# lvclark/tagdigger

Measured on AMD Instinct MI355X. Metric: FASTQ reads/sec (whole node), 200M-read × 100k-tag synthetic, 1/2/4/8 MI355X, higher is better.
Workload: dtype u8; 1 GPU; BASELINE configs[2] shape, device-resident (tier T1): 200000000 reads x 384 barcodes x 100000 tags per GPU, 100 bp reads, 219 B/record, cut site TGCAG, one library per GPU; reads_per_gpu=200000000, barcodes=384, tags=100000, fastq_bytes_per_gpu=43800000000

## Files before the change

tagdigger_amd/csrc/inst_fast4.hip:

```cpp
#include <hip/hip_runtime.h>
#define TD_INST_ONLY 1
#include "kernel_fast4.hpp"
#define X(W, NQ) template __global__ void tdk::k_fast4<W, NQ, (TD_INST_PROG != 0)>(const tdk::FParams);
TD_FAST2_COMBOS(X)
#undef X
```

tagdigger_amd/csrc/kernel_fast4.hpp:

```cpp
#pragma once
#include "kernel_fast2.hpp"

namespace tdk {

#ifndef TD_F4_WAVES
#define TD_F4_WAVES 16
#endif
#ifndef TD_F4_NPROD
#define TD_F4_NPROD 11
#endif
#ifndef TD_F4_SLOTS
#define TD_F4_SLOTS 5
#endif
constexpr int F4_PROD = 4 , F4_WAVES = TD_F4_WAVES, F4_BLOCK = 64 * F4_WAVES;
#ifndef TD_F4_CPT
#define TD_F4_CPT 6
#endif
constexpr int F4_CPT = TD_F4_CPT;
constexpr uint32_t F4_WCH = F4_CPT * 64;
constexpr uint32_t F4_WBYTES = F4_WCH * 16;
constexpr uint32_t F4_TILE = F4_PROD * F4_WBYTES;
constexpr int F4_SLOTS = TD_F4_SLOTS;
constexpr uint32_t F4_SPIN_LIMIT = 1u << 18;
#ifndef TD_F4_EAGER_MIN
#define TD_F4_EAGER_MIN 65
#endif
#ifndef TD_F4_EAGER_SPINS
#define TD_F4_EAGER_SPINS 4
#endif
#ifndef TD_F4_P_CONS
#define TD_F4_P_CONS 1
#endif

enum { F4_DONE = 0, F4_FREE = 1, F4_REMAIN = 2, F4_FLAGS = 3, F4_TOT = 4 , F4_VOTE = 8 , F4_R0 = 12, F4_WB1 = 13, F4_WB2 = 14,
       F4_WB3 = 15, F4_TOTAL = 16, F4_SEQ = 17, F4_NCUM = 18, F4_NWANT = 19, F4_TIDX = 20, F4_CTRL_DW = 24 };
constexpr uint32_t F4_FLAG_HI = 1, F4_FLAG_OVER = 2, F4_FLAG_HALO_HI = 4;
constexpr uint32_t F4_ABORT_DW = F4_SLOTS * F4_CTRL_DW, F4_READY_DW = F4_ABORT_DW + 1, F4_AVAIL_DW = F4_ABORT_DW + 2, F4_CLAIMED_DW = F4_ABORT_DW + 3;
constexpr uint32_t F4_NPROD_MIN = 7, F4_NPROD_MAX = 13;
constexpr uint32_t F4_CTRL_BYTES = 1024;
static_assert(F4_CLAIMED_DW < 240 && F4_WAVES <= 16, "hand-off words");

__device__ __forceinline__ uint32_t lds_ld(const uint32_t *p) { return __hip_atomic_load(p, __ATOMIC_RELAXED, __HIP_MEMORY_SCOPE_WORKGROUP); }
__device__ __forceinline__ void lds_st(uint32_t *p, uint32_t v) { __hip_atomic_store(p, v, __ATOMIC_RELAXED, __HIP_MEMORY_SCOPE_WORKGROUP); }
__device__ __forceinline__ bool f4_wait(uint32_t *p, uint32_t need, uint32_t *abort_word, unsigned long long *stats) {
    for (uint32_t spins = 0;; spins++) {
        const uint32_t v = lds_ld(p);
        if (v >= need) break;
        if (spins > F4_SPIN_LIMIT || lds_ld(abort_word)) {
            lds_st(abort_word, 1u);
            if ((threadIdx.x & 63) == 0) atomicOr(stats + ST_ERR, ERR_SPIN);
            return false;
        }
        __builtin_amdgcn_s_sleep(1);
    }
    asm volatile("s_waitcnt lgkmcnt(0)" ::: "memory");
    return true;
}

#ifndef TD_INST_ONLY
__global__ __launch_bounds__(256) void k_f4_estimate(const uint8_t *buf, uint64_t nbytes, uint32_t *out) {
    __shared__ uint32_t total;
    if (threadIdx.x == 0) total = 0;
    __syncthreads();
    const uint32_t n = (uint32_t)(nbytes < 65536ull ? nbytes : 65536ull) & ~15u;
    uint32_t cnt = 0;
    for (uint32_t i = threadIdx.x * 16u; i < n; i += 256u * 16u) {
        const uint4 v = *reinterpret_cast<const uint4 *>(buf + i);
        cnt += (uint32_t)__builtin_popcount(eq_mask16(v, 0x0A0A0A0Au) | eq_mask16(v, 0x0D0D0D0Du));
    }
    atomicAdd(&total, cnt);
    __syncthreads();
    if (threadIdx.x == 0) {
        const uint32_t rec = total >= 8u ? 4u * n / total : 219u;
        *out = rec < 150u ? 8u : rec < 195u ? 9u : rec < 270u ? 10u : rec < 420u ? 11u : 12u;
    }
}
#endif

#ifdef TD_PHASE_PROF
#define F4_STAMP(i) do { const unsigned long long now_ = __builtin_amdgcn_s_memtime(); f4acc[i] += now_ - f4last; f4last = now_; } while (0)
#else
#define F4_STAMP(i) do {} while (0)
#endif

template <int W, int NQ, bool PROG>
__global__ __launch_bounds__(F4_BLOCK, F4_WAVES / 4) void k_fast4(const FParams fp) {
    const KParams &p = fp.k;
#ifdef TD_PHASE_PROF
    unsigned long long f4acc[12] = {};
    unsigned long long f4last = __builtin_amdgcn_s_memtime();
#endif
    constexpr uint32_t TILE = F4_TILE, WCH = F4_WCH, WBYTES = F4_WBYTES;
    constexpr int CPT = F4_CPT;
    static_assert(W <= 3, "k_fast4 has the pipelined probe of the 64-byte buckets only");

    extern __shared__ __attribute__((aligned(16))) uint8_t lds[];
    const uint32_t halo = p.halo;
    const uint32_t slot_bytes = TILE + halo;
    uint8_t *L_raw0 = lds;
    uint16_t *L_list0 = reinterpret_cast<uint16_t *>(lds + F4_SLOTS * slot_bytes);
    uint32_t *L_ctrl = reinterpret_cast<uint32_t *>(lds + F4_SLOTS * slot_bytes + F4_SLOTS * F4_PROD * WCH * 2u);
    uint32_t *L_abort = L_ctrl + F4_ABORT_DW;
    uint8_t *L_hc = reinterpret_cast<uint8_t *>(L_ctrl) + F4_CTRL_BYTES;
    uint8_t *L_bidx = L_hc + ((uint32_t)F4_WAVES - F4_NPROD_MIN) * HC_BYTES_PER_WAVE;
    TileCtx cx{nullptr, 0u, reinterpret_cast<const unsigned long long *>(L_bidx),
               reinterpret_cast<const uint32_t *>(L_bidx + p.off_bmeta),
               reinterpret_cast<const uint16_t *>(L_bidx + p.off_bdir)};

    const int tid = threadIdx.x, lane = tid & 63;
    const int wave = __builtin_amdgcn_readfirstlane(tid >> 6);
    for (uint32_t i = tid; i < p.bblob_bytes / 4; i += F4_BLOCK)
        reinterpret_cast<uint32_t *>(L_bidx)[i] = p.bblob[i];
    if (tid < (int)(F4_CTRL_BYTES / 4)) L_ctrl[tid] = 0;
    __syncthreads();

    const unsigned long long carried = p.cursor_in ? *p.cursor_in : 0ull;
    const uint64_t first_line = p.first_line + carried;
    const uint32_t nwork = p.ntiles;
    const uint32_t RUN = p.run ? p.run : 1u;
    auto tile_base = [&](uint32_t tile) -> const uint8_t * {
        return tile >= p.tail_tile ? p.tail_buf + (uint64_t)(tile - p.tail_tile) * TILE : p.buf + (uint64_t)tile * TILE;
    };
    typedef uint32_t u32x4 __attribute__((ext_vector_type(4)));
    auto tile_rsrc = [&](uint32_t tile) {
        return __builtin_amdgcn_make_buffer_rsrc(const_cast<uint8_t *>(tile_base(tile)), 0, (int)(TILE + 4096u), 0x00020000);
    };

    uint32_t np_ = p.f4_nprod ? p.f4_nprod : (p.f4_nprod_dev ? *p.f4_nprod_dev : (uint32_t)TD_F4_NPROD);
    np_ = np_ < F4_NPROD_MIN ? F4_NPROD_MIN : np_ > F4_NPROD_MAX ? F4_NPROD_MAX : np_;
    const uint32_t NPROD = (uint32_t)__builtin_amdgcn_readfirstlane((int)np_);
    {
        uint4 va[CPT], vb[CPT];
        u32x4 vha, vhb;
        auto fetch_job = [&](uint4 (&v)[CPT], u32x4 &vh, uint32_t tile, uint32_t q) {
            const uint32_t voff = q * WBYTES + (uint32_t)lane * 16u;
            const bool hh = q == (uint32_t)F4_PROD - 1u && (uint32_t)lane < halo / 16u;
            const uint32_t hoff = hh ? (uint32_t)lane * 16u : 0x40000000u;
            const __amdgpu_buffer_rsrc_t rs = tile_rsrc(tile);
#pragma unroll
            for (int j = 0; j < CPT; j++) {
                const u32x4 qq = __builtin_amdgcn_raw_buffer_load_b128(rs, voff, j * 1024, 2 );
                v[j] = make_uint4(qq.x, qq.y, qq.z, qq.w);
            }
            vh = __builtin_amdgcn_raw_buffer_load_b128(rs, hoff, (int)TILE, 0);
        };
        auto tile_of = [&](uint32_t k) -> uint32_t { return (k / RUN) * (gridDim.x * RUN) + blockIdx.x * RUN + k % RUN; };
        uint32_t n_local = 0;
        for (uint32_t first = blockIdx.x * RUN; first < nwork; first += gridDim.x * RUN) n_local += min(RUN, nwork - first);
        uint32_t my_job = (uint32_t)wave;
        if (wave < (int)NPROD) {
            if (my_job < 4u * n_local) fetch_job(va, vha, tile_of(my_job >> 2), my_job & 3u);
            if (my_job + NPROD < 4u * n_local) fetch_job(vb, vhb, tile_of((my_job + NPROD) >> 2), (my_job + NPROD) & 3u);
        }
        uint32_t *g_ready = L_ctrl + F4_READY_DW, *g_avail = L_ctrl + F4_AVAIL_DW, *g_claimed = L_ctrl + F4_CLAIMED_DW;

        if (wave < (int)NPROD) {
        auto produce = [&](uint4 (&v)[CPT], u32x4 &vh, const uint32_t k, const uint32_t t) -> bool {
            const uint32_t qtr = my_job & 3u;
            const uint32_t voff = qtr * WBYTES + (uint32_t)lane * 16u;
            const bool has_halo = qtr == (uint32_t)F4_PROD - 1u && (uint32_t)lane < halo / 16u;
            const uint32_t slot = k % (uint32_t)F4_SLOTS, use = k / (uint32_t)F4_SLOTS;
            uint8_t *L_raw = L_raw0 + slot * slot_bytes;
            uint16_t *Ll = L_list0 + (slot * F4_PROD + qtr) * WCH;
            uint32_t *ctrl = L_ctrl + slot * F4_CTRL_DW;
            const uint64_t tbase = (uint64_t)t * TILE;
            const bool carry_ok = k % RUN != 0u && t != 1u;
            const uint32_t job2 = my_job + 2u * NPROD;
            const bool more = job2 < 4u * n_local;
            const uint32_t t2 = more ? tile_of(job2 >> 2) : 0u;
            F4_STAMP(4);
            if (!f4_wait(ctrl + F4_FREE, use, L_abort, p.stats)) return false;
            F4_STAMP(0);
            bool wave_crb = false;
            uint32_t myflags = 0;
            {
                uint32_t hiacc = 0;
#pragma unroll
                for (int j = 0; j < CPT; j++) hiacc |= v[j].x | v[j].y | v[j].z | v[j].w;
#pragma unroll
                for (int j = 0; j < CPT; j++) *reinterpret_cast<uint4 *>(L_raw + voff + j * 1024) = v[j];
                uint16_t *Lm = Ll + lane;
                const bool general = __any((hiacc & 0x80808080u) != 0);
                if (__builtin_expect(!general, 1)) {
                    uint32_t cr_absent = 0x80808080u;
#pragma unroll
                    for (int j = 0; j < CPT; j++) cr_absent_ascii(v[j], cr_absent);
                    const bool has_cr = __any((cr_absent & 0x80808080u) != 0x80808080u);
                    if (__builtin_expect(!has_cr, 1)) {
#pragma unroll
                        for (int j = 0; j < CPT; j++) Lm[j * 64] = (uint16_t)nl_mask16_ascii(v[j]);
                    } else {
                        uint32_t crs = 0;
#pragma unroll
                        for (int j = 0; j < CPT; j++) {
                            const uint32_t nl = eq_mask16_ascii(v[j], 0x0A0A0A0Au, 0x7F7F7F7Fu), cr = eq_mask16_ascii(v[j], 0x0D0D0D0Du, 0x7F7F7F7Fu);
// ... 2 lines not shown
                        }
                        wave_crb = __any((crs & 0x8000u) != 0);
                    }
                } else {
                    uint32_t crs = 0;
#pragma unroll
                    for (int j = 0; j < CPT; j++) {
                        const uint32_t nl = eq_mask16(v[j], 0x0A0A0A0Au), cr = eq_mask16(v[j], 0x0D0D0D0Du);
                        Lm[j * 64] = (uint16_t)(nl | (cr & ~(nl >> 1)));
                        crs |= cr;
                    }
                    wave_crb = __any((crs & 0x8000u) != 0);
                    myflags |= F4_FLAG_HI;
                }
            }
            if (has_halo) *reinterpret_cast<uint4 *>(L_raw + TILE + (uint32_t)lane * 16u) = make_uint4(vh.x, vh.y, vh.z, vh.w);
            if (qtr == (uint32_t)F4_PROD - 1u && __any(has_halo && ((vh.x | vh.y | vh.z | vh.w) & 0x80808080u) != 0)) myflags |= F4_FLAG_HALO_HI;
            const uint32_t my_qtr = qtr;
            if (more) fetch_job(v, vh, t2, job2 & 3u);
            wave_lds_fence();
            F4_STAMP(1);

            uint32_t mm[CPT / 2];
#pragma unroll
            for (int i = 0; i < CPT / 2; i++) mm[i] = reinterpret_cast<const uint32_t *>(Ll)[lane * (CPT / 2) + i];
            const uint32_t span0 = my_qtr * WBYTES + (uint32_t)lane * (CPT * 16u);
            const uint32_t wend = (my_qtr + 1u) * WBYTES;
            if (__builtin_expect(wave_crb, 0)) {
#pragma unroll
                for (int i = 0; i < CPT / 2; i++) {
#pragma unroll
                    for (int hbit = 15; hbit < 32; hbit += 16) {
                        if ((mm[i] >> hbit) & 1u) {
                            const uint32_t at = span0 + 32u * i + (uint32_t)hbit;
                            if (L_raw[at] == 0x0Du) {
                                const uint32_t nx = at + 1u < wend ? (uint32_t)L_raw[at + 1u] : (uint32_t)tile_base(t)[at + 1u];
                                if (nx == 0x0Au) mm[i] &= ~(1u << hbit);
                            }
                        }
                    }
                }
            }
            uint32_t cnt = 0;
#pragma unroll
            for (int i = 0; i < CPT / 2; i++) cnt += __builtin_popcount(mm[i]);
            const uint32_t incl = wave_incl_scan(cnt, lane);
            const uint32_t wtot = (uint32_t)__builtin_amdgcn_readlane((int)incl, 63);
            uint32_t packed = 0;
            if (!carry_ok) {
                uint32_t fpos = 0;
                bool found = false;
// ... 90 lines not shown
                asm volatile("s_waitcnt lgkmcnt(0)" ::: "memory");
                if (lane == 0)
                    __hip_atomic_store(reinterpret_cast<unsigned long long *>(ctrl + F4_NCUM), (unsigned long long)ncum | ((unsigned long long)nwant << 32),
                                       __ATOMIC_RELAXED, __HIP_MEMORY_SCOPE_WORKGROUP);
                asm volatile("s_waitcnt lgkmcnt(0)" ::: "memory");
                if (lane == 0) {
                    lds_st(g_avail, ncum + nwant);
                    if (nwant == 0u) lds_st(ctrl + F4_FREE, use + 1u);
                }
                asm volatile("s_waitcnt lgkmcnt(0)" ::: "memory");
                if (lane == 0) lds_st(g_ready, k + 1u);
                F4_STAMP(3);
            }
            return true;
        };
            for (;;) {
                if (!(my_job < 4u * n_local)) break;
                if (!produce(va, vha, my_job >> 2, tile_of(my_job >> 2))) break;
                my_job += NPROD;
                if (!(my_job < 4u * n_local)) break;
                if (!produce(vb, vhb, my_job >> 2, tile_of(my_job >> 2))) break;
                my_job += NPROD;
            }
        } else {
        const int cons = wave < (int)NPROD ? 0 : wave - (int)NPROD;
        uint2 *hcS = reinterpret_cast<uint2 *>(L_hc + cons * HC_BYTES_PER_WAVE);
        uint8_t *hcE = L_hc + cons * HC_BYTES_PER_WAVE + HC_SLOTS * 8;
        if (wave >= (int)NPROD) {
#pragma unroll
            for (int q = 0; q < HC_SLOTS / 64; q++) hcS[q * 64 + lane] = make_uint2(HC_EMPTY, 0u);
            wave_lds_fence();
        }
        bool hc_on = p.hot_cache != 0;
        uint32_t hc_hits = 0, hc_rest = 0, aged = 0;
        int st_reads = 0, st_bar = 0, st_tag = 0;
        Pending<W> pd;
        Pending<W> nx;
        bool pd_valid = false;
        bool phit_tag = false;
        auto finish_pending = [&](bool &hit, uint32_t &cell) {
            vm_settled();
            const uint64_t res = match_finish<W>(p, pd);
            const uint32_t kind = (uint32_t)(res >> 62);
// ... 146 lines not shown
                    break;
                }
                __builtin_amdgcn_s_sleep(1);
            }
            settle();
            if (p.hot_cache) hc_flush(p.counts, hcS, (uint32_t)lane);
            unsigned long long r = wave_sum64((unsigned long long)(long long)st_reads), b = wave_sum64((unsigned long long)(long long)st_bar),
                               g = wave_sum64((unsigned long long)(long long)st_tag);
            if (lane == 0) {
                if (r) atomicAdd(p.stats + ST_READS, r);
                if (b) atomicAdd(p.stats + ST_BARCUT, b);
                if (g) atomicAdd(p.stats + ST_TAG, g);
            }
        }
#ifdef TD_PHASE_PROF
        if (lane == 0) for (int i = 0; i < 9; i++) atomicAdd(p.stats + 8 + i, f4acc[i]);
#endif
    }
}

}

#ifdef TD_FAST4_EXTERN
#define TD_X4(W, NQ) extern template __global__ void tdk::k_fast4<W, NQ, false>(const tdk::FParams); extern template __global__ void tdk::k_fast4<W, NQ, true>(const tdk::FParams);
TD_FAST2_COMBOS(TD_X4)
#undef TD_X4
#endif
```

tagdigger_amd/csrc/kernels.hpp:

```cpp
#pragma once
#include <hip/hip_runtime.h>
#include <stdint.h>

namespace tdk {

constexpr int BLOCK = 256;
constexpr int TLIST_CAP = 2048;
constexpr int LBQ = 4;
constexpr uint64_t FLAG_AGG = 1ull << 62;
constexpr uint64_t FLAG_INC = 2ull << 62;
constexpr uint64_t VAL_MASK = (1ull << 62) - 1;
constexpr uint32_t BDIR_BASES = 5;
constexpr uint32_t BDIR_SIZE = 1u << (2 * BDIR_BASES);
#ifndef TD_BU4
#define TD_BU4 4
#endif
constexpr uint32_t BMETA_LAST = 1u << 12;
constexpr uint32_t SPIN_LIMIT = 1u << 22;
constexpr uint64_t R_NONE = 0, R_BAR = 1ull << 62, R_TAG = 2ull << 62, R_DEFER = 3ull << 62, R_CELL = (1ull << 62) - 1;
constexpr int IPL = 4;

constexpr uint32_t DBG_NO_ATOMIC = 1, DBG_NO_PROBE = 2, DBG_NO_PHASE2 = 4, DBG_NO_LOOKBACK = 8,
                   DBG_NO_PACK = 16, DBG_STATIC_TILES = 32;

// ... 25 lines not shown
    uint32_t prefilled;
    const unsigned long long *cursor_in;
    unsigned long long *cursor_out;
    uint32_t nt_loads;
    const uint8_t *tail_buf;
    uint32_t tail_tile;
    uint32_t prio;
    uint32_t stagger, stagger_div;
    uint32_t dbg;
    uint32_t hot_cache;
    uint32_t run;
    unsigned long long *win;
    uint32_t win_cap;
    uint32_t f4_nprod;
    const uint32_t *f4_nprod_dev;
};
constexpr uint32_t PROG_WINDOW = 50000;

__device__ __forceinline__ uint32_t udot4(uint32_t a, uint32_t b, uint32_t c) {
    return __builtin_amdgcn_udot4(a, b, c, false);
}
__device__ __forceinline__ uint32_t eq_bytes(uint32_t x, uint32_t c4) {
    uint32_t y = x ^ c4;
    uint32_t t = ((y & 0x7F7F7F7Fu) + 0x7F7F7F7Fu) | y | 0x7F7F7F7Fu;
    return (~t) >> 7;
}
__device__ __forceinline__ uint32_t eq_mask16(const uint4 &v, uint32_t c4) {
    uint32_t lo = udot4(eq_bytes(v.x, c4), 0x08040201u, 0u);
    lo = udot4(eq_bytes(v.y, c4), 0x80402010u, lo);
    uint32_t hi = udot4(eq_bytes(v.z, c4), 0x08040201u, 0u);
// ... 785 lines not shown
```

tagdigger_amd/csrc/tagdig.hip:

```cpp
#include <hip/hip_runtime.h>
#include <fcntl.h>
#include <sys/stat.h>
#include <unistd.h>
#include <zlib.h>

#include <algorithm>
#include <atomic>
#include <condition_variable>
#include <cstdio>
#include <cstring>
#include <mutex>
#include <string>
#include <chrono>
#include <thread>
#include <unordered_map>
#include <vector>

#include "../../include/tagdig.h"
#include "../../include/td_synth_spec.h"
#include "kernels.hpp"
#include "kernel_fast.hpp"
#define TD_FAST2_EXTERN 1
#include "kernel_fast2.hpp"
#define TD_FAST4_EXTERN 1
// ... 193 lines not shown
    int gz_gpu_verify = 0;
    uint32_t gz_gpu_seg_kb = 1u << 20, gz_gpu_margin_kb = 16384;
    int gz_gpu_false_every = 0;
    int gpu_resolve = 1;
    uint8_t *d_zscratch = nullptr; uint32_t *d_crctab = nullptr;
    uint32_t zcap_members = 0; size_t zcap_in = 0;
    int gpu_inflate = 1;
    int gpu_inflate_crc = 1;
    uint32_t max_need = 0;
    int tile_kb = 32, blocks_per_cu = 0, prescan = 0, timing = 0, fastpath = 1, nt_loads = 1;
    int kernel_gen = 4;
    int tile_kb2 = 0;
    int run = 8;
    int hot_cache = 1;
    int f4_nprod = 0;
    uint64_t fast_max_matrix = 1ull << 32;
    uint32_t debug_ablate = 0;
    double table_load = 0.25;
    int stagger = 0;
    int prio = 0xE4;
    std::vector<std::pair<hipEvent_t, hipEvent_t>> ev_pool;
    size_t ev_used = 0;
    const void *occ_fn = nullptr; size_t occ_lds = 0; int occ_val = 1;
};

namespace {

void release_bgzf_buffers(td_handle *h) {
    for (auto &zp : h->zpiece) {
        if (zp.pin) (void)hipHostFree(zp.pin);
// ... 58 lines not shown
    switch (W) {
    case 1: return nq == 3 ? tdk::k_fast2<CPT, 1, 3, PROG> : nq == 4 ? tdk::k_fast2<CPT, 1, 4, PROG> : tdk::k_fast2<CPT, 1, 6, PROG>;
    case 2: return nq == 5 ? tdk::k_fast2<CPT, 2, 5, PROG> : nq == 6 ? tdk::k_fast2<CPT, 2, 6, PROG> : tdk::k_fast2<CPT, 2, 8, PROG>;
    default: return nq == 7 ? tdk::k_fast2<CPT, 3, 7, PROG> : nq == 8 ? tdk::k_fast2<CPT, 3, 8, PROG> : tdk::k_fast2<CPT, 3, 10, PROG>;
    }
}
FFn pick_fast2(int tile_kb, int W, uint32_t nq, bool prog) {
    if (prog) return tile_kb == 32 ? pick_fast2_c<8, true>(W, nq) : tile_kb == 24 ? pick_fast2_c<6, true>(W, nq) : pick_fast2_c<4, true>(W, nq);
    return tile_kb == 32 ? pick_fast2_c<8, false>(W, nq) : tile_kb == 24 ? pick_fast2_c<6, false>(W, nq) : pick_fast2_c<4, false>(W, nq);
}
FFn pick_fix(int tile_kb, int W) {
    if (tile_kb == 24) return pick_fast_w<6, true>(W);
    if (tile_kb == 12) return W == 1 ? tdk::k_fast<6, 1, true, 128> : W == 2 ? tdk::k_fast<6, 2, true, 128> : tdk::k_fast<6, 3, true, 128>;
    return pick_fast(tile_kb, W, true);
}
template <bool PROG> FFn pick_fast4_p(int W, uint32_t nq) {
    switch (W) {
    case 1: return nq == 3 ? tdk::k_fast4<1, 3, PROG> : nq == 4 ? tdk::k_fast4<1, 4, PROG> : tdk::k_fast4<1, 6, PROG>;
    case 2: return nq == 5 ? tdk::k_fast4<2, 5, PROG> : nq == 6 ? tdk::k_fast4<2, 6, PROG> : tdk::k_fast4<2, 8, PROG>;
    default: return nq == 7 ? tdk::k_fast4<3, 7, PROG> : nq == 8 ? tdk::k_fast4<3, 8, PROG> : tdk::k_fast4<3, 10, PROG>;
    }
}
FFn pick_fast4(int W, uint32_t nq, bool prog) { return prog ? pick_fast4_p<true>(W, nq) : pick_fast4_p<false>(W, nq); }
size_t lds_bytes_fast4(const td_handle *h) {
    return (size_t)tdk::F4_SLOTS * (tdk::F4_TILE + h->halo) + (size_t)tdk::F4_SLOTS * tdk::F4_PROD * tdk::F4_WCH * 2 + tdk::F4_CTRL_BYTES +
           (size_t)(tdk::F4_WAVES - tdk::F4_NPROD_MIN) * tdk::HC_BYTES_PER_WAVE + h->bblob_bytes;
}
int fast2_auto_tile(const td_handle *h);
size_t lds_bytes_fast2(const td_handle *h, int tile_kb) {
    const size_t tile = (size_t)tile_kb * 1024;
    return tile + h->halo + tile / 16 * 2 + 256 + 4 * tdk::HC_BYTES_PER_WAVE + h->bblob_bytes;
}

int fast2_auto_tile(const td_handle *h) {
    if (lds_bytes_fast2(h, 24) <= 160 * 1024 / 4) return 24;
    if (lds_bytes_fast2(h, 32) <= 160 * 1024 / 3) return 32;
    if (lds_bytes_fast2(h, 24) <= LDS_BUDGET) return 24;
    return 16;
}

size_t lds_bytes_fast(const td_handle *h, int tile_kb) {
// ... 35 lines not shown
int launch_count(td_handle *h, const void *d_fastq, uint64_t nbytes, uint64_t first_line, uint64_t max_reads,
                 int weights, hipStream_t stream, const unsigned long long *cursor_in = nullptr,
                 unsigned long long *cursor_out = nullptr, uint64_t first_line_ub = 0) {
    if (h->sink) return h->sink->piece(h->sink->ctx, d_fastq, nbytes, first_line, max_reads, stream, cursor_in, cursor_out);
    if (!h->have_index) return fail(TD_E_STATE, "td_set_index has not been called");
    if (((uintptr_t)d_fastq & 15) != 0) return fail(TD_E_ARG, "device FASTQ pointer must be 16-byte aligned");
    if (nbytes == 0) return TD_OK;
    if (max_reads == 0) max_reads = 1;
    h->counted = true;
    const bool tassel = weights != 0;
    const uint64_t limit_line = max_reads >= (1ull << 60) ? ~0ull - 8 : 4 * (max_reads - 1) + 1;
    const uint64_t fl_ub = std::max(first_line, first_line_ub);
    const bool limit_far = limit_line >= ~0ull - 16 || limit_line - std::min(limit_line, fl_ub) >= nbytes / 16;
    const bool counts32 = (uint64_t)h->barnum * h->ntags * 4 < h->fast_max_matrix;
    const int tkb2 = h->tile_kb2 ? h->tile_kb2 : fast2_auto_tile(h);
    const bool gen4_fits = h->kernel_gen == 4 && h->W <= 3 && lds_bytes_fast4(h) <= 160 * 1024;
    const bool gen2_fits = (h->kernel_gen == 2 || (h->kernel_gen == 4 && !gen4_fits)) && h->W <= 3 && lds_bytes_fast2(h, tkb2) <= LDS_BUDGET;
    const bool use_fast = h->fastpath && !tassel && !h->prescan && limit_far && counts32 && !(h->progress && !gen2_fits && !gen4_fits);
    const bool gen4 = use_fast && gen4_fits;
    const bool gen2 = use_fast && gen2_fits && !gen4;
    const int tile_kb = tassel ? 16 : gen4 ? (int)(tdk::F4_TILE / 1024) : gen2 ? tkb2 : h->tile_kb;
    const uint64_t tile = (uint64_t)tile_kb * 1024;
    const uint64_t ntiles64 = (nbytes + tile - 1) / tile;
    if (ntiles64 > 0x7FFFFFFFull) return fail(TD_E_LIMIT, "buffer too large for one launch; split it");
    const uint32_t ntiles = (uint32_t)ntiles64;

    if (!h->bound_counts && !tassel) {
        if ((h->bytes_since_flush + nbytes) / 4 >= h->flush_limit) { int rc = flush_counts(h); if (rc) return rc; }
        h->bytes_since_flush += nbytes;
    }
    if (tassel) {
        if (!h->d_counts64.p) {
            int rc = h->d_counts64.ensure((size_t)h->barnum * h->ntags); if (rc) return rc;
            HIPCHK(hipMemsetAsync(h->d_counts64.p, 0, (size_t)h->barnum * h->ntags * 8, stream));
        }
// ... 9 lines not shown
    p.off_bdir = h->off_bdir; p.off_bcand = h->off_bcand;
    p.buckets = h->d_slots.p; p.bucket_mask = h->bucket_mask; p.m_bases = h->m_bases;
    p.shorts = h->d_shorts.p; p.nshort = h->nshort;
    p.counts = h->bound_counts ? h->bound_counts : h->d_counts.p; p.counts64 = h->d_counts64.p;
    p.ncols = h->ntags; p.stats = h->d_stats.p; p.nch = h->nch; p.maxwo = h->maxwo;
    p.prefilled = h->prescan ? 1u : 0u;
    p.cursor_in = cursor_in; p.cursor_out = cursor_out;
    p.dbg = h->debug_ablate;
    p.stagger = (uint32_t)h->stagger; p.stagger_div = (uint32_t)h->num_cu;
    p.nt_loads = (uint32_t)h->nt_loads;
    p.prio = (uint32_t)h->prio;

    p.hot_cache = (uint32_t)h->hot_cache;
    p.run = (uint32_t)h->run;
    p.f4_nprod = (uint32_t)h->f4_nprod;
    if (h->progress) {
        const uint64_t need = (fl_ub + nbytes) / 4 / tdk::PROG_WINDOW + 2;
        if (need > h->d_win.n) {
            const size_t cap = (size_t)std::max<uint64_t>(need * 2, 1u << 16);
            DevBuf<unsigned long long> bigger;
            int rc = bigger.ensure(cap); if (rc) return rc;
            HIPCHK(hipStreamSynchronize(stream));
            HIPCHK(hipMemset(bigger.p, 0, cap * 8));
            if (h->d_win.p) HIPCHK(hipMemcpy(bigger.p, h->d_win.p, h->d_win.n * 8, hipMemcpyDeviceToDevice));
            h->d_win.release();
            h->d_win = bigger;
        }
        p.win = h->d_win.p; p.win_cap = (uint32_t)std::min<size_t>(h->d_win.n, 0xFFFFFFFFu);
    }
    h->last_fast_tile_kb = use_fast ? tile_kb : 0;
// ... 11 lines not shown
            const uint64_t start = inside * TILE;
            if (nbytes - start > tail_cap) return fail(TD_E_INTERNAL, "tail copy larger than its buffer");
            HIPCHK(hipMemsetAsync(h->d_tail.p, 0, tail_cap, stream));
            if (nbytes > start)
                HIPCHK(hipMemcpyAsync(h->d_tail.p, (const uint8_t *)d_fastq + start, nbytes - start, hipMemcpyDeviceToDevice, stream));
            p.tail_buf = h->d_tail.p; p.tail_tile = (uint32_t)inside;
        }
        tdk::FParams fp{};
        fp.k = p; fp.tile_info = h->d_tileinfo.p; fp.fixlist = h->d_fixlist.p; fp.nfix = h->d_nfix.p; fp.fix_cap = fix_cap;
        if (h->progress) {
            rc = h->d_tilesums.ensure(ntiles); if (rc) return rc;
            HIPCHK(hipMemsetAsync(h->d_tilesums.p, 0, (size_t)ntiles * 4, stream));
            fp.tile_sums = h->d_tilesums.p;
        }
        HIPCHK(hipMemsetAsync(h->d_nfix.p, 0, 4, stream));
        FFn ffn = gen4 ? pick_fast4(h->W, h->nch2, h->progress != 0) : gen2 ? pick_fast2(tile_kb, h->W, h->nch2, h->progress != 0) : pick_fast(tile_kb, h->W, false), fixfn = pick_fix(tile_kb, h->W);
        const size_t flds = gen4 ? lds_bytes_fast4(h) : gen2 ? lds_bytes_fast2(h, tile_kb) : lds_bytes_fast(h, tile_kb), fixlds = lds_bytes_fast(h, tile_kb);
        const unsigned main_threads = gen4 ? (unsigned)tdk::F4_BLOCK : (unsigned)tdk::FBLOCK, fix_threads = tile_kb == 12 ? 128u : (unsigned)tdk::FBLOCK;
        if (flds > 48 * 1024) HIPCHK(hipFuncSetAttribute((const void *)ffn, hipFuncAttributeMaxDynamicSharedMemorySize, (int)flds));
        if (fixlds > 48 * 1024) HIPCHK(hipFuncSetAttribute((const void *)fixfn, hipFuncAttributeMaxDynamicSharedMemorySize, (int)fixlds));
        int bpc = h->blocks_per_cu;
        if (bpc <= 0) {
            if (h->occ_fn != (const void *)ffn || h->occ_lds != flds) {
                int occ = 0;
                HIPCHK(hipOccupancyMaxActiveBlocksPerMultiprocessor(&occ, (const void *)ffn, (int)main_threads, flds));
                h->occ_fn = (const void *)ffn; h->occ_lds = flds; h->occ_val = std::max(1, occ);
            }
            bpc = h->occ_val;
        }
        const uint32_t grid = (uint32_t)std::min<uint64_t>(ntiles, (uint64_t)h->num_cu * bpc);
        hipEvent_t e0 = nullptr, e1 = nullptr;
        if (h->timing) {
            if (h->ev_used == h->ev_pool.size()) {
                hipEvent_t a, b;
                HIPCHK(hipEventCreate(&a)); HIPCHK(hipEventCreate(&b));
                h->ev_pool.emplace_back(a, b);
            }
            e0 = h->ev_pool[h->ev_used].first; e1 = h->ev_pool[h->ev_used].second; h->ev_used++;
            HIPCHK(hipEventRecord(e0, stream));
        }
        if (gen4 && !h->f4_nprod) {
            int rc4 = h->d_f4np.ensure(4); if (rc4) return rc4;
            hipLaunchKernelGGL(tdk::k_f4_estimate, dim3(1), dim3(256), 0, stream, (const uint8_t *)d_fastq, nbytes, h->d_f4np.p);
            fp.k.f4_nprod_dev = h->d_f4np.p;
        }
        hipLaunchKernelGGL(ffn, dim3(grid), dim3(main_threads), flds, stream, fp);
        {
            const uint32_t rblocks = (ntiles + tdk::RESOLVE_SPAN - 1) / tdk::RESOLVE_SPAN;
            unsigned long long *super = reinterpret_cast<unsigned long long *>(h->d_state.p);
            hipLaunchKernelGGL(tdk::k_resolve_sums, dim3(rblocks), dim3(256), 0, stream, fp, super);
            hipLaunchKernelGGL(tdk::k_resolve, dim3(rblocks), dim3(1024), 0, stream, fp, super);
        }
        hipLaunchKernelGGL(fixfn, dim3(std::min<uint32_t>(grid, (uint32_t)h->num_cu * 2)), dim3(fix_threads), fixlds, stream, fp);
        HIPCHK(hipGetLastError());
        if (h->timing) HIPCHK(hipEventRecord(e1, stream));
        return TD_OK;
// ... 1995 lines not shown
        for (size_t i = 0; i < cells; i++) out[i] += t64[i];
    }
    return TD_OK;
}

int td_debug_counters(td_handle *h, uint64_t out[24]) {
    if (!h || !out) return fail(TD_E_ARG, "NULL argument");
    HIPCHK(hipSetDevice(h->device));
    HIPCHK(hipDeviceSynchronize());
    HIPCHK(hipMemcpy(out, h->d_stats.p + 8, 24 * 8, hipMemcpyDeviceToHost));
    if (h->d_nfix.p) {
        uint32_t nf = 0;
        HIPCHK(hipMemcpy(&nf, h->d_nfix.p, 4, hipMemcpyDeviceToHost));
        out[11] = nf;
    }
    return TD_OK;
}

int td_set_option(td_handle *h, const char *name, int64_t value) {
    if (!h || !name) return fail(TD_E_ARG, "NULL argument");
    std::string n(name);
    if (n == "tile_kb") {
        if (value != 16 && value != 32) return fail(TD_E_ARG, "tile_kb must be 16 or 32");
        if (h->have_index && lds_bytes(h, (int)value) > LDS_BUDGET) return fail(TD_E_LIMIT, "tile does not fit the LDS budget with this index");
        h->tile_kb = (int)value;
    } else if (n == "blocks_per_cu") h->blocks_per_cu = (int)value;
    else if (n == "prescan") h->prescan = value ? 1 : 0;
    else if (n == "timing") h->timing = value ? 1 : 0;
    else if (n == "fastpath") h->fastpath = value ? 1 : 0;
    else if (n == "kernel") {
        if (value != 1 && value != 2 && value != 4) return fail(TD_E_ARG, "kernel must be 1 (k_fast), 2 (k_fast2) or 4 (k_fast4)");
        h->kernel_gen = (int)value;
    } else if (n == "tile_kb2") {
        if (value != 0 && value != 16 && value != 24 && value != 32) return fail(TD_E_ARG, "tile_kb2 must be 0 (automatic), 16, 24 or 32");
        if (value && h->have_index && lds_bytes_fast2(h, (int)value) > LDS_BUDGET) return fail(TD_E_LIMIT, "tile does not fit the LDS budget with this index");
        h->tile_kb2 = (int)value;
    } else if (n == "f4_nprod") {
        if (value != 0 && (value < tdk::F4_NPROD_MIN || value > tdk::F4_NPROD_MAX)) return fail(TD_E_ARG, "f4_nprod: 7 .. 13 producer waves of k_fast4's sixteen (0: from the input's line density)");
        h->f4_nprod = (int)value;
    } else if (n == "hot_cache") h->hot_cache = value == 2 ? 2 : value ? 1 : 0;
    else if (n == "run") h->run = (int)std::max<int64_t>(1, std::min<int64_t>(value, 4096));
    else if (n == "progress") h->progress = value ? 1 : 0;
    else if (n == "zb_members") h->zb_members = (uint32_t)std::max<int64_t>(64, value);
    else if (n == "split_kernel") h->split_kernel = value == 1 ? 1 : 2;
    else if (n == "gpu_huffman") h->gpu_huffman = value ? 1 : 0;
    else if (n == "gz_gpu_min") h->gz_gpu_min = (uint64_t)std::max<long long>(0, value);
    else if (n == "md5_piece") { if (value < 0 || value % 64) return fail(TD_E_ARG, "md5_piece: a multiple of 64, or 0"); h->md5_piece = (uint64_t)value; }
    else if (n == "tagnet_max_compares") { if (value < 0) return fail(TD_E_ARG, "tagnet_max_compares: 0 or more"); h->tagnet_max_compares = (uint64_t)value; }
    else if (n == "gz_gpu_terr_kb") { if (value < 16 || value > 4096) return fail(TD_E_ARG, "gz_gpu_terr_kb: 16..4096"); h->gz_gpu_terr_kb = (uint32_t)value; }
    else if (n == "gz_gpu_release") { h->gzgpu.release(); }
    else if (n == "gz_gpu_verify") h->gz_gpu_verify = value ? 1 : 0;
    else if (n == "gz_gpu_seg_kb") { if (value < 64 || value > (4 << 20)) return fail(TD_E_ARG, "gz_gpu_seg_kb: 64..4194304"); h->gz_gpu_seg_kb = (uint32_t)value; }
    else if (n == "gz_gpu_margin_kb") { if (value < 64 || value > (1 << 20)) return fail(TD_E_ARG, "gz_gpu_margin_kb: 64..1048576"); h->gz_gpu_margin_kb = (uint32_t)value; }
    else if (n == "gz_gpu_false_every") h->gz_gpu_false_every = (int)std::max<long long>(0, value);
// ... 943 lines not shown
```

Baseline: 18.64 billion reads/s.

## Add dedicated loader waves that DMA tiles straight into LDS for k_fast4

Result: slower. 17.28 billion reads/s (-7.3%).

```diff
diff --git a/tagdigger_amd/csrc/inst_fast4.hip b/tagdigger_amd/csrc/inst_fast4.hip
--- a/tagdigger_amd/csrc/inst_fast4.hip
+++ b/tagdigger_amd/csrc/inst_fast4.hip
@@ -1,6 +1,9 @@
 #include <hip/hip_runtime.h>
 #define TD_INST_ONLY 1
 #include "kernel_fast4.hpp"
-#define X(W, NQ) template __global__ void tdk::k_fast4<W, NQ, (TD_INST_PROG != 0)>(const tdk::FParams);
+#ifndef TD_INST_LDR
+#define TD_INST_LDR 0
+#endif
+#define X(W, NQ) template __global__ void tdk::k_fast4<W, NQ, (TD_INST_PROG != 0), (TD_INST_LDR != 0)>(const tdk::FParams);
 TD_FAST2_COMBOS(X)
 #undef X
diff --git a/tagdigger_amd/csrc/kernel_fast4.hpp b/tagdigger_amd/csrc/kernel_fast4.hpp
--- a/tagdigger_amd/csrc/kernel_fast4.hpp
+++ b/tagdigger_amd/csrc/kernel_fast4.hpp
@@ -33,10 +33,14 @@
 #endif
 
 enum { F4_DONE = 0, F4_FREE = 1, F4_REMAIN = 2, F4_FLAGS = 3, F4_TOT = 4 , F4_VOTE = 8 , F4_R0 = 12, F4_WB1 = 13, F4_WB2 = 14,
-       F4_WB3 = 15, F4_TOTAL = 16, F4_SEQ = 17, F4_NCUM = 18, F4_NWANT = 19, F4_TIDX = 20, F4_CTRL_DW = 24 };
+       F4_WB3 = 15, F4_TOTAL = 16, F4_SEQ = 17, F4_NCUM = 18, F4_NWANT = 19, F4_TIDX = 20, F4_LANDED = 21 , F4_CTRL_DW = 24 };
 constexpr uint32_t F4_FLAG_HI = 1, F4_FLAG_OVER = 2, F4_FLAG_HALO_HI = 4;
 constexpr uint32_t F4_ABORT_DW = F4_SLOTS * F4_CTRL_DW, F4_READY_DW = F4_ABORT_DW + 1, F4_AVAIL_DW = F4_ABORT_DW + 2, F4_CLAIMED_DW = F4_ABORT_DW + 3;
 constexpr uint32_t F4_NPROD_MIN = 7, F4_NPROD_MAX = 13;
+constexpr uint32_t F4_NSCAN_MIN = 4, F4_NSCAN_MAX = 12;
+constexpr uint32_t F4_HC_WAVES = F4_WAVES - F4_NPROD_MIN, F4L_HC_WAVES = F4_WAVES - 1 - F4_NSCAN_MIN;
+constexpr uint32_t F4L_PIECES = F4_TILE / 1024u + 1u;
+static_assert(2u * F4L_PIECES <= 63u, "two tiles in flight behind a counted s_waitcnt: vmcnt has six bits");
 constexpr uint32_t F4_CTRL_BYTES = 1024;
 static_assert(F4_CLAIMED_DW < 240 && F4_WAVES <= 16, "hand-off words");
 
@@ -57,6 +61,7 @@
     return true;
 }
 
+__host__ __device__ inline uint32_t f4_scanners_for(uint32_t rec) { return rec < 150u ? 5u : rec < 270u ? 6u : rec < 420u ? 7u : 8u; }
 #ifndef TD_INST_ONLY
 __global__ __launch_bounds__(256) void k_f4_estimate(const uint8_t *buf, uint64_t nbytes, uint32_t *out) {
     __shared__ uint32_t total;
@@ -73,6 +78,7 @@
     if (threadIdx.x == 0) {
         const uint32_t rec = total >= 8u ? 4u * n / total : 219u;
         *out = rec < 150u ? 8u : rec < 195u ? 9u : rec < 270u ? 10u : rec < 420u ? 11u : 12u;
+        out[1] = f4_scanners_for(rec);
     }
 }
 #endif
@@ -83,7 +89,7 @@
 #define F4_STAMP(i) do {} while (0)
 #endif
 
-template <int W, int NQ, bool PROG>
+template <int W, int NQ, bool PROG, bool LDR = false>
 __global__ __launch_bounds__(F4_BLOCK, F4_WAVES / 4) void k_fast4(const FParams fp) {
     const KParams &p = fp.k;
 #ifdef TD_PHASE_PROF
@@ -102,7 +108,7 @@
     uint32_t *L_ctrl = reinterpret_cast<uint32_t *>(lds + F4_SLOTS * slot_bytes + F4_SLOTS * F4_PROD * WCH * 2u);
     uint32_t *L_abort = L_ctrl + F4_ABORT_DW;
     uint8_t *L_hc = reinterpret_cast<uint8_t *>(L_ctrl) + F4_CTRL_BYTES;
-    uint8_t *L_bidx = L_hc + ((uint32_t)F4_WAVES - F4_NPROD_MIN) * HC_BYTES_PER_WAVE;
+    uint8_t *L_bidx = L_hc + (LDR ? F4L_HC_WAVES : F4_HC_WAVES) * HC_BYTES_PER_WAVE;
     TileCtx cx{nullptr, 0u, reinterpret_cast<const unsigned long long *>(L_bidx),
                reinterpret_cast<const uint32_t *>(L_bidx + p.off_bmeta),
                reinterpret_cast<const uint16_t *>(L_bidx + p.off_bdir)};
@@ -128,7 +134,14 @@
 
     uint32_t np_ = p.f4_nprod ? p.f4_nprod : (p.f4_nprod_dev ? *p.f4_nprod_dev : (uint32_t)TD_F4_NPROD);
     np_ = np_ < F4_NPROD_MIN ? F4_NPROD_MIN : np_ > F4_NPROD_MAX ? F4_NPROD_MAX : np_;
+    if constexpr (LDR) {
+        np_ = p.f4_nscan ? p.f4_nscan : p.f4_nprod ? p.f4_nprod - (p.f4_nload == 2u ? 2u : 1u) : (p.f4_nprod_dev ? p.f4_nprod_dev[1] : 8u);
+        np_ = np_ < F4_NSCAN_MIN ? F4_NSCAN_MIN : np_ > F4_NSCAN_MAX ? F4_NSCAN_MAX : np_;
+    }
     const uint32_t NPROD = (uint32_t)__builtin_amdgcn_readfirstlane((int)np_);
+    const uint32_t NLOAD = LDR ? (uint32_t)__builtin_amdgcn_readfirstlane((int)(p.f4_nload == 2u ? 2u : 1u)) : 0u;
+    const int jwave = wave - (int)NLOAD;
+    const uint32_t NNM = NPROD + NLOAD;
     {
         uint4 va[CPT], vb[CPT];
         u32x4 vha, vhb;
@@ -147,14 +160,51 @@
         auto tile_of = [&](uint32_t k) -> uint32_t { return (k / RUN) * (gridDim.x * RUN) + blockIdx.x * RUN + k % RUN; };
         uint32_t n_local = 0;
         for (uint32_t first = blockIdx.x * RUN; first < nwork; first += gridDim.x * RUN) n_local += min(RUN, nwork - first);
-        uint32_t my_job = (uint32_t)wave;
-        if (wave < (int)NPROD) {
+        uint32_t my_job = (uint32_t)jwave;
+        if (!LDR && wave < (int)NPROD) {
             if (my_job < 4u * n_local) fetch_job(va, vha, tile_of(my_job >> 2), my_job & 3u);
             if (my_job + NPROD < 4u * n_local) fetch_job(vb, vhb, tile_of((my_job + NPROD) >> 2), (my_job + NPROD) & 3u);
         }
         uint32_t *g_ready = L_ctrl + F4_READY_DW, *g_avail = L_ctrl + F4_AVAIL_DW, *g_claimed = L_ctrl + F4_CLAIMED_DW;
 
-        if (wave < (int)NPROD) {
+        if (LDR && wave < (int)NLOAD) {
+            typedef __attribute__((address_space(3))) uint8_t lds_byte;
+            const uint32_t L_base = (uint32_t)__builtin_amdgcn_readfirstlane((int)(uint32_t)(uintptr_t)(lds_byte *)L_raw0);
+            auto dma_piece = [&](const u32x4 rs, const uint32_t dst, const uint32_t soff) {
+                uint32_t keep;
+                asm volatile("s_mov_b32 %0, m0\n\ts_mov_b32 m0, %1\n\ts_nop 0\n\tbuffer_load_dwordx4 %2, %3, %4 offen nt lds\n\ts_mov_b32 m0, %0"
+                             : "=&s"(keep) : "s"(dst), "v"((uint32_t)lane * 16u), "s"(rs), "s"(soff) : "memory");
+            };
+            __builtin_amdgcn_s_setprio(3);
+            uint32_t landed = (uint32_t)wave;
+            auto publish = [&](const uint32_t upto) {
+                for (; landed < upto; landed += NLOAD)
+                    if (lane == 0) lds_st(L_ctrl + (landed % (uint32_t)F4_SLOTS) * F4_CTRL_DW + F4_LANDED, landed / (uint32_t)F4_SLOTS + 1u);
+            };
+            for (uint32_t k = (uint32_t)wave; k < n_local; k += NLOAD) {
+                const uint32_t slot = k % (uint32_t)F4_SLOTS, use = k / (uint32_t)F4_SLOTS;
+                uint32_t *ctrl = L_ctrl + slot * F4_CTRL_DW;
+                F4_STAMP(4);
+                if (lds_ld(ctrl + F4_FREE) < use) {
+                    asm volatile("s_waitcnt vmcnt(0)" ::: "memory");
+                    publish(k);
+                    if (!f4_wait(ctrl + F4_FREE, use, L_abort, p.stats)) break;
+                }
+                F4_STAMP(9);
+                const uint64_t ta = (uint64_t)tile_base(tile_of(k));
+                const u32x4 rs = {(uint32_t)__builtin_amdgcn_readfirstlane((int)(uint32_t)ta),
+                                  (uint32_t)__builtin_amdgcn_readfirstlane((int)(uint32_t)(ta >> 32)) & 0xFFFFu, TILE + 4096u, 0x00020000u};
+                const uint32_t dst = L_base + slot * (uint32_t)__builtin_amdgcn_readfirstlane((int)slot_bytes);
+#pragma unroll
+                for (uint32_t j = 0; j < TILE / 1024u; j++) dma_piece(rs, dst + j * 1024u, j * 1024u);
+                if ((uint32_t)lane < halo / 16u) dma_piece(rs, dst + TILE, TILE);
+                asm volatile("s_waitcnt vmcnt(%0)" :: "n"(F4L_PIECES) : "memory");
+                publish(k);
+                F4_STAMP(10);
+            }
+            asm volatile("s_waitcnt vmcnt(0)" ::: "memory");
+            publish(n_local);
+        } else if (wave < (int)NNM) {
         auto produce = [&](uint4 (&v)[CPT], u32x4 &vh, const uint32_t k, const uint32_t t) -> bool {
             const uint32_t qtr = my_job & 3u;
             const uint32_t voff = qtr * WBYTES + (uint32_t)lane * 16u;
@@ -166,10 +216,18 @@
             const uint64_t tbase = (uint64_t)t * TILE;
             const bool carry_ok = k % RUN != 0u && t != 1u;
             const uint32_t job2 = my_job + 2u * NPROD;
-            const bool more = job2 < 4u * n_local;
+            const bool more = !LDR && job2 < 4u * n_local;
             const uint32_t t2 = more ? tile_of(job2 >> 2) : 0u;
             F4_STAMP(4);
-            if (!f4_wait(ctrl + F4_FREE, use, L_abort, p.stats)) return false;
+            if constexpr (LDR) {
+                if (!f4_wait(ctrl + F4_LANDED, use + 1u, L_abort, p.stats)) return false;
+#pragma unroll
+                for (int j = 0; j < CPT; j++) v[j] = *reinterpret_cast<const uint4 *>(L_raw + voff + j * 1024);
+                vh = u32x4{0u, 0u, 0u, 0u};
+                if (has_halo) vh = *reinterpret_cast<const u32x4 *>(L_raw + TILE + (uint32_t)lane * 16u);
+            } else {
+                if (!f4_wait(ctrl + F4_FREE, use, L_abort, p.stats)) return false;
+            }
             F4_STAMP(0);
             bool wave_crb = false;
             uint32_t myflags = 0;
@@ -178,7 +236,7 @@
 #pragma unroll
                 for (int j = 0; j < CPT; j++) hiacc |= v[j].x | v[j].y | v[j].z | v[j].w;
 #pragma unroll
-                for (int j = 0; j < CPT; j++) *reinterpret_cast<uint4 *>(L_raw + voff + j * 1024) = v[j];
+                for (int j = 0; j < CPT; j++) if (!LDR) *reinterpret_cast<uint4 *>(L_raw + voff + j * 1024) = v[j];
                 uint16_t *Lm = Ll + lane;
                 const bool general = __any((hiacc & 0x80808080u) != 0);
                 if (__builtin_expect(!general, 1)) {
@@ -211,7 +269,7 @@
                     myflags |= F4_FLAG_HI;
                 }
             }
-            if (has_halo) *reinterpret_cast<uint4 *>(L_raw + TILE + (uint32_t)lane * 16u) = make_uint4(vh.x, vh.y, vh.z, vh.w);
+            if (!LDR && has_halo) *reinterpret_cast<uint4 *>(L_raw + TILE + (uint32_t)lane * 16u) = make_uint4(vh.x, vh.y, vh.z, vh.w);
             if (qtr == (uint32_t)F4_PROD - 1u && __any(has_halo && ((vh.x | vh.y | vh.z | vh.w) & 0x80808080u) != 0)) myflags |= F4_FLAG_HALO_HI;
             const uint32_t my_qtr = qtr;
             if (more) fetch_job(v, vh, t2, job2 & 3u);
@@ -231,7 +289,7 @@
                         if ((mm[i] >> hbit) & 1u) {
                             const uint32_t at = span0 + 32u * i + (uint32_t)hbit;
                             if (L_raw[at] == 0x0Du) {
-                                const uint32_t nx = at + 1u < wend ? (uint32_t)L_raw[at + 1u] : (uint32_t)tile_base(t)[at + 1u];
+                                const uint32_t nx = LDR || at + 1u < wend ? (uint32_t)L_raw[at + 1u] : (uint32_t)tile_base(t)[at + 1u];
                                 if (nx == 0x0Au) mm[i] &= ~(1u << hbit);
                             }
                         }
@@ -352,6 +410,8 @@
             }
             return true;
         };
+            if (LDR && p.f4_sprio == 1u) __builtin_amdgcn_s_setprio(1);
+            if (LDR && p.f4_sprio == 2u) __builtin_amdgcn_s_setprio(2);
             for (;;) {
                 if (!(my_job < 4u * n_local)) break;
                 if (!produce(va, vha, my_job >> 2, tile_of(my_job >> 2))) break;
@@ -361,10 +421,10 @@
                 my_job += NPROD;
             }
         } else {
-        const int cons = wave < (int)NPROD ? 0 : wave - (int)NPROD;
+        const int cons = wave < (int)NNM ? 0 : wave - (int)NNM;
         uint2 *hcS = reinterpret_cast<uint2 *>(L_hc + cons * HC_BYTES_PER_WAVE);
         uint8_t *hcE = L_hc + cons * HC_BYTES_PER_WAVE + HC_SLOTS * 8;
-        if (wave >= (int)NPROD) {
+        if (wave >= (int)NNM) {
 #pragma unroll
             for (int q = 0; q < HC_SLOTS / 64; q++) hcS[q * 64 + lane] = make_uint2(HC_EMPTY, 0u);
             wave_lds_fence();
@@ -541,7 +601,7 @@
             }
         }
 #ifdef TD_PHASE_PROF
-        if (lane == 0) for (int i = 0; i < 9; i++) atomicAdd(p.stats + 8 + i, f4acc[i]);
+        if (lane == 0) for (int i = 0; i < 11; i++) atomicAdd(p.stats + 8 + i, f4acc[i]);
 #endif
     }
 }
@@ -549,7 +609,8 @@
 }
 
 #ifdef TD_FAST4_EXTERN
-#define TD_X4(W, NQ) extern template __global__ void tdk::k_fast4<W, NQ, false>(const tdk::FParams); extern template __global__ void tdk::k_fast4<W, NQ, true>(const tdk::FParams);
+#define TD_X4(W, NQ) extern template __global__ void tdk::k_fast4<W, NQ, false, false>(const tdk::FParams); extern template __global__ void tdk::k_fast4<W, NQ, true, false>(const tdk::FParams); \
+    extern template __global__ void tdk::k_fast4<W, NQ, false, true>(const tdk::FParams); extern template __global__ void tdk::k_fast4<W, NQ, true, true>(const tdk::FParams);
 TD_FAST2_COMBOS(TD_X4)
 #undef TD_X4
 #endif
diff --git a/tagdigger_amd/csrc/kernels.hpp b/tagdigger_amd/csrc/kernels.hpp
--- a/tagdigger_amd/csrc/kernels.hpp
+++ b/tagdigger_amd/csrc/kernels.hpp
@@ -63,6 +63,9 @@
     uint32_t win_cap;
     uint32_t f4_nprod;
     const uint32_t *f4_nprod_dev;
+    uint32_t f4_nload;
+    uint32_t f4_sprio;
+    uint32_t f4_nscan;
 };
 constexpr uint32_t PROG_WINDOW = 50000;
 
diff --git a/tagdigger_amd/csrc/tagdig.hip b/tagdigger_amd/csrc/tagdig.hip
--- a/tagdigger_amd/csrc/tagdig.hip
+++ b/tagdigger_amd/csrc/tagdig.hip
@@ -231,6 +231,11 @@
     int run = 8;
     int hot_cache = 1;
     int f4_nprod = 0;
+    int f4_loader = 1;
+    int f4_nload = 1;
+    int f4_sprio = 0;
+    int f4_nscan = 0;
+    int last_main_pass = 0;
     uint64_t fast_max_matrix = 1ull << 32;
     uint32_t debug_ablate = 0;
     double table_load = 0.25;
@@ -319,17 +324,19 @@
     if (tile_kb == 12) return W == 1 ? tdk::k_fast<6, 1, true, 128> : W == 2 ? tdk::k_fast<6, 2, true, 128> : tdk::k_fast<6, 3, true, 128>;
     return pick_fast(tile_kb, W, true);
 }
-template <bool PROG> FFn pick_fast4_p(int W, uint32_t nq) {
+template <bool PROG, bool LDR> FFn pick_fast4_p(int W, uint32_t nq) {
     switch (W) {
-    case 1: return nq == 3 ? tdk::k_fast4<1, 3, PROG> : nq == 4 ? tdk::k_fast4<1, 4, PROG> : tdk::k_fast4<1, 6, PROG>;
-    case 2: return nq == 5 ? tdk::k_fast4<2, 5, PROG> : nq == 6 ? tdk::k_fast4<2, 6, PROG> : tdk::k_fast4<2, 8, PROG>;
-    default: return nq == 7 ? tdk::k_fast4<3, 7, PROG> : nq == 8 ? tdk::k_fast4<3, 8, PROG> : tdk::k_fast4<3, 10, PROG>;
-    }
-}
-FFn pick_fast4(int W, uint32_t nq, bool prog) { return prog ? pick_fast4_p<true>(W, nq) : pick_fast4_p<false>(W, nq); }
-size_t lds_bytes_fast4(const td_handle *h) {
+    case 1: return nq == 3 ? tdk::k_fast4<1, 3, PROG, LDR> : nq == 4 ? tdk::k_fast4<1, 4, PROG, LDR> : tdk::k_fast4<1, 6, PROG, LDR>;
+    case 2: return nq == 5 ? tdk::k_fast4<2, 5, PROG, LDR> : nq == 6 ? tdk::k_fast4<2, 6, PROG, LDR> : tdk::k_fast4<2, 8, PROG, LDR>;
+    default: return nq == 7 ? tdk::k_fast4<3, 7, PROG, LDR> : nq == 8 ? tdk::k_fast4<3, 8, PROG, LDR> : tdk::k_fast4<3, 10, PROG, LDR>;
+    }
+}
+FFn pick_fast4(int W, uint32_t nq, bool prog, bool loader) {
+    return loader ? (prog ? pick_fast4_p<true, true>(W, nq) : pick_fast4_p<false, true>(W, nq)) : (prog ? pick_fast4_p<true, false>(W, nq) : pick_fast4_p<false, false>(W, nq));
+}
+size_t lds_bytes_fast4(const td_handle *h, bool loader) {
     return (size_t)tdk::F4_SLOTS * (tdk::F4_TILE + h->halo) + (size_t)tdk::F4_SLOTS * tdk::F4_PROD * tdk::F4_WCH * 2 + tdk::F4_CTRL_BYTES +
-           (size_t)(tdk::F4_WAVES - tdk::F4_NPROD_MIN) * tdk::HC_BYTES_PER_WAVE + h->bblob_bytes;
+           (size_t)(loader ? tdk::F4L_HC_WAVES : tdk::F4_HC_WAVES) * tdk::HC_BYTES_PER_WAVE + h->bblob_bytes;
 }
 int fast2_auto_tile(const td_handle *h);
 size_t lds_bytes_fast2(const td_handle *h, int tile_kb) {
@@ -395,11 +402,14 @@
     const bool limit_far = limit_line >= ~0ull - 16 || limit_line - std::min(limit_line, fl_ub) >= nbytes / 16;
     const bool counts32 = (uint64_t)h->barnum * h->ntags * 4 < h->fast_max_matrix;
     const int tkb2 = h->tile_kb2 ? h->tile_kb2 : fast2_auto_tile(h);
-    const bool gen4_fits = h->kernel_gen == 4 && h->W <= 3 && lds_bytes_fast4(h) <= 160 * 1024;
+    const bool gen4l_fits = h->kernel_gen == 4 && h->f4_loader && h->W <= 3 && lds_bytes_fast4(h, true) <= 160 * 1024;
+    const bool gen4_fits = gen4l_fits || (h->kernel_gen == 4 && h->W <= 3 && lds_bytes_fast4(h, false) <= 160 * 1024);
     const bool gen2_fits = (h->kernel_gen == 2 || (h->kernel_gen == 4 && !gen4_fits)) && h->W <= 3 && lds_bytes_fast2(h, tkb2) <= LDS_BUDGET;
     const bool use_fast = h->fastpath && !tassel && !h->prescan && limit_far && counts32 && !(h->progress && !gen2_fits && !gen4_fits);
     const bool gen4 = use_fast && gen4_fits;
     const bool gen2 = use_fast && gen2_fits && !gen4;
+    const bool gen4l = gen4 && gen4l_fits;
+    h->last_main_pass = gen4l ? 5 : gen4 ? 4 : gen2 ? 2 : use_fast ? 1 : 0;
     const int tile_kb = tassel ? 16 : gen4 ? (int)(tdk::F4_TILE / 1024) : gen2 ? tkb2 : h->tile_kb;
     const uint64_t tile = (uint64_t)tile_kb * 1024;
     const uint64_t ntiles64 = (nbytes + tile - 1) / tile;
@@ -439,6 +449,9 @@
     p.hot_cache = (uint32_t)h->hot_cache;
     p.run = (uint32_t)h->run;
     p.f4_nprod = (uint32_t)h->f4_nprod;
+    p.f4_nscan = (uint32_t)h->f4_nscan;
+    p.f4_nload = (uint32_t)h->f4_nload;
+    p.f4_sprio = (uint32_t)h->f4_sprio;
     if (h->progress) {
         const uint64_t need = (fl_ub + nbytes) / 4 / tdk::PROG_WINDOW + 2;
         if (need > h->d_win.n) {
@@ -480,8 +493,8 @@
             fp.tile_sums = h->d_tilesums.p;
         }
         HIPCHK(hipMemsetAsync(h->d_nfix.p, 0, 4, stream));
-        FFn ffn = gen4 ? pick_fast4(h->W, h->nch2, h->progress != 0) : gen2 ? pick_fast2(tile_kb, h->W, h->nch2, h->progress != 0) : pick_fast(tile_kb, h->W, false), fixfn = pick_fix(tile_kb, h->W);
-        const size_t flds = gen4 ? lds_bytes_fast4(h) : gen2 ? lds_bytes_fast2(h, tile_kb) : lds_bytes_fast(h, tile_kb), fixlds = lds_bytes_fast(h, tile_kb);
+        FFn ffn = gen4 ? pick_fast4(h->W, h->nch2, h->progress != 0, gen4l) : gen2 ? pick_fast2(tile_kb, h->W, h->nch2, h->progress != 0) : pick_fast(tile_kb, h->W, false), fixfn = pick_fix(tile_kb, h->W);
+        const size_t flds = gen4 ? lds_bytes_fast4(h, gen4l) : gen2 ? lds_bytes_fast2(h, tile_kb) : lds_bytes_fast(h, tile_kb), fixlds = lds_bytes_fast(h, tile_kb);
         const unsigned main_threads = gen4 ? (unsigned)tdk::F4_BLOCK : (unsigned)tdk::FBLOCK, fix_threads = tile_kb == 12 ? 128u : (unsigned)tdk::FBLOCK;
         if (flds > 48 * 1024) HIPCHK(hipFuncSetAttribute((const void *)ffn, hipFuncAttributeMaxDynamicSharedMemorySize, (int)flds));
         if (fixlds > 48 * 1024) HIPCHK(hipFuncSetAttribute((const void *)fixfn, hipFuncAttributeMaxDynamicSharedMemorySize, (int)fixlds));
@@ -505,7 +518,7 @@
             e0 = h->ev_pool[h->ev_used].first; e1 = h->ev_pool[h->ev_used].second; h->ev_used++;
             HIPCHK(hipEventRecord(e0, stream));
         }
-        if (gen4 && !h->f4_nprod) {
+        if (gen4 && !h->f4_nprod && !(gen4l && h->f4_nscan)) {
             int rc4 = h->d_f4np.ensure(4); if (rc4) return rc4;
             hipLaunchKernelGGL(tdk::k_f4_estimate, dim3(1), dim3(256), 0, stream, (const uint8_t *)d_fastq, nbytes, h->d_f4np.p);
             fp.k.f4_nprod_dev = h->d_f4np.p;
@@ -2531,6 +2544,7 @@
         HIPCHK(hipMemcpy(&nf, h->d_nfix.p, 4, hipMemcpyDeviceToHost));
         out[11] = nf;
     }
+    out[12] = (uint64_t)h->last_main_pass;
     return TD_OK;
 }
 
@@ -2555,6 +2569,15 @@
     } else if (n == "f4_nprod") {
         if (value != 0 && (value < tdk::F4_NPROD_MIN || value > tdk::F4_NPROD_MAX)) return fail(TD_E_ARG, "f4_nprod: 7 .. 13 producer waves of k_fast4's sixteen (0: from the input's line density)");
         h->f4_nprod = (int)value;
+    } else if (n == "f4_loader") h->f4_loader = value ? 1 : 0;
+    else if (n == "f4_sprio") h->f4_sprio = (int)std::max<int64_t>(0, std::min<int64_t>(value, 2));
+    else if (n == "f4_nload") {
+        if (value != 1 && value != 2) return fail(TD_E_ARG, "f4_nload: 1 or 2 loader waves of k_fast4's loader form");
+        h->f4_nload = (int)value;
+    }
+    else if (n == "f4_nscan") {
+        if (value != 0 && (value < tdk::F4_NSCAN_MIN || value > tdk::F4_NSCAN_MAX)) return fail(TD_E_ARG, "f4_nscan: 4 .. 12 scanner waves of k_fast4's loader form (0: from f4_nprod, else from the input's line density)");
+        h->f4_nscan = (int)value;
     } else if (n == "hot_cache") h->hot_cache = value == 2 ? 2 : value ? 1 : 0;
     else if (n == "run") h->run = (int)std::max<int64_t>(1, std::min<int64_t>(value, 4096));
     else if (n == "progress") h->progress = value ? 1 : 0;
```
